# ArielElb/zkSnark-FinalProject

Measured on AMD Instinct MI355X. Metric: groth16_proofs_per_sec, higher is better.
Workload: dtype u32; 1 GPU; matrix-mul 128x128 + Poseidon MatrixCircuit: 10706932 constraints, 8675313 witness vars, domain 2^24; pk/R1CS/assignment resident in HBM; real key (zkg16_setup_resident) with window tables (zkg16_pk_precompute), last timed proof verified (zkg16_verify); parallelism=1 GPU

## Files before the change

zksnark-finalproject_amd/csrc/api.hip:

```cpp
#include <chrono>
#include <functional>
#include <thread>

#include <exception>

#include "common.hpp"
#include "group.hpp"

using namespace zk;

namespace zk {
ScopedKernelTimer::ScopedKernelTimer(zkg16_ctx *c, const char *n, double u, hipStream_t st)
    : ctx(c), name(n), units(u), stream(st ? st : c->stream) {
    if (!ctx->kernel_timing) return;
    if (ctx->kernel_timing_accumulate_only && strncmp(n, "msm_accumulate", 14) != 0) return;
    ZK_HIP(hipEventCreate(&e0));
    ZK_HIP(hipEventCreate(&e1));
    ZK_HIP(hipEventRecord(e0, stream));
}
ScopedKernelTimer::~ScopedKernelTimer() {
    if (!e0) return;
    (void)hipEventRecord(e1, stream);
    ctx->pending_events.push_back(PendingEvent{name, units, e0, e1});
}
// ... 31 lines not shown
    if (e.err == hipErrorInvalidValue && strstr(e.what, "domain")) return ZKG16_ERR_DOMAIN_TOO_LARGE;
    return ZKG16_ERR_HIP;
}

#define ZK_API_BEGIN(ctx)                         \
    if (!(ctx)) return ZKG16_ERR_BAD_ARG;         \
    std::lock_guard<std::mutex> _lk((ctx)->mu);   \
    try {                                         \
        ZK_HIP(hipSetDevice((ctx)->device));
#define ZK_API_END(ctx)                           \
    }                                             \
    catch (const HipError &e) { return fail((ctx), e); } \
    catch (const std::bad_alloc &) { return ZKG16_ERR_OOM; } \
    return ZKG16_OK;

void copy_options(zkg16_ctx *dst, const zkg16_ctx *src) {
    dst->opt_window_bits = src->opt_window_bits; dst->opt_min_seg = src->opt_min_seg; dst->opt_ntt_mode = src->opt_ntt_mode;
    dst->opt_reduce_mode = src->opt_reduce_mode; dst->opt_b_filter = src->opt_b_filter; dst->opt_spmv_dict = src->opt_spmv_dict;
    dst->opt_wm_first = src->opt_wm_first; dst->opt_g1_waves = src->opt_g1_waves; dst->opt_fixup_aux = src->opt_fixup_aux;
    dst->opt_window_bits_h = src->opt_window_bits_h; dst->opt_reduce_chunk = src->opt_reduce_chunk; dst->opt_wm_concurrent = src->opt_wm_concurrent;
    dst->opt_ntt_radix = src->opt_ntt_radix; dst->opt_ntt_xcd = src->opt_ntt_xcd; dst->opt_acc_debug = src->opt_acc_debug;
    dst->opt_sort_mode = src->opt_sort_mode; dst->opt_acc_pipeline = src->opt_acc_pipeline; dst->opt_fuse_pointwise = src->opt_fuse_pointwise;
    dst->opt_matrix_parts = src->opt_matrix_parts; dst->opt_g2_lazy = src->opt_g2_lazy; dst->opt_g1_inline = src->opt_g1_inline; dst->opt_fixed_base_bits = src->opt_fixed_base_bits;
    dst->opt_collect_threads = src->opt_collect_threads; dst->opt_batch_max = src->opt_batch_max; dst->opt_matrix_batch_threads = src->opt_matrix_batch_threads; dst->opt_matrix_batch_grid = src->opt_matrix_batch_grid; dst->opt_verify_batch_min = src->opt_verify_batch_min; dst->opt_verify_wire_min = src->opt_verify_wire_min; dst->opt_verify_each_after = src->opt_verify_each_after; dst->opt_wm_transforms = src->opt_wm_transforms;
    dst->kernel_timing = src->kernel_timing; dst->kernel_timing_accumulate_only = src->kernel_timing_accumulate_only;
}
void create_streams(zkg16_ctx *ctx) {
    ZK_HIP(hipStreamCreateWithFlags(&ctx->stream, hipStreamNonBlocking));
    ZK_HIP(hipStreamCreateWithFlags(&ctx->wm_stream, hipStreamNonBlocking));
    for (int i : {0, 2, 3, 4, 1}) ZK_HIP(hipStreamCreateWithFlags(&ctx->slots[i].stream, hipStreamNonBlocking));
}
void teardown(zkg16_ctx *ctx) {
    (void)hipStreamSynchronize(ctx->stream);
    (void)hipStreamSynchronize(ctx->wm_stream);
    if (ctx->extra_host) (void)hipHostFree(ctx->extra_host);
    if (ctx->batch_host) (void)hipHostFree(ctx->batch_host);
    ctx->batch_host = nullptr;
    ctx->batch_host_bytes = 0;
    if (ctx->mbatch_host) (void)hipHostFree(ctx->mbatch_host);
    ctx->mbatch_host = nullptr;
    ctx->mbatch_host_bytes = 0;
    ctx->mbatch_dev.release();
    if (ctx->circuit_stage) (void)hipHostFree(ctx->circuit_stage);
    ctx->circuit_stage = nullptr;
    ctx->circuit_stage_bytes = 0;
    for (int i = 0; i < 2; i++) {
        if (ctx->stage_host[i]) (void)hipHostFree(ctx->stage_host[i]);
// ... 939 lines not shown
        if (value < 0 || value > 15) return ZKG16_ERR_BAD_ARG;
        ctx->opt_acc_debug = (int)value;
        return ZKG16_OK;
    }
    if (!strcmp(name, "sort_mode")) {
        if (value < 0 || value > 1) return ZKG16_ERR_BAD_ARG;
        ctx->opt_sort_mode = (int)value;
        return ZKG16_OK;
    }
    if (!strcmp(name, "acc_pipeline")) {
        if (value < 0 || value > 4) return ZKG16_ERR_BAD_ARG;
        ctx->opt_acc_pipeline = value == 4 ? 0 : (int)value;
        return ZKG16_OK;
    }
    if (!strcmp(name, "fuse_pointwise")) {
        ctx->opt_fuse_pointwise = value ? 1 : 0;
        return ZKG16_OK;
    }
    if (!strcmp(name, "wm_transforms")) {
        if (value != 0 && value != 6 && value != 7) return ZKG16_ERR_BAD_ARG;
        ctx->opt_wm_transforms = value == 7 ? 7 : 6;
        return ZKG16_OK;
    }
    if (!strcmp(name, "wm_first")) {
        if (value < -1 || value > 2) return ZKG16_ERR_BAD_ARG;
        ctx->opt_wm_first = (int)value;
        return ZKG16_OK;
    }
    if (!strcmp(name, "spmv_dict")) {
        if (value < 0 || value > 2) return ZKG16_ERR_BAD_ARG;
        ctx->opt_spmv_dict = (int)value;
        return ZKG16_OK;
    }
    if (!strcmp(name, "b_filter")) {
        if (value < 0 || value > 2) return ZKG16_ERR_BAD_ARG;
        ctx->opt_b_filter = (int)value;
        return ZKG16_OK;
    }
    if (!strcmp(name, "collect_threads")) {
        if (value < 0 || value > 2) return ZKG16_ERR_BAD_ARG;
        ctx->opt_collect_threads = value == 0 ? -1 : value == 2 ? 0 : 1;
        return ZKG16_OK;
    }
    if (!strcmp(name, "fixed_base_bits")) {
        if (value != 0 && (value < 4 || value > 20 || (value > 14 && (value & 1)))) return ZKG16_ERR_BAD_ARG;
        ctx->opt_fixed_base_bits = (int)value;
// ... 1750 lines not shown
```

zksnark-finalproject_amd/csrc/common.hpp:

```cpp
#pragma once
#include <hip/hip_runtime.h>
#include <stdint.h>
#include <stdio.h>
#include <string.h>

#include <algorithm>
#include <array>
#include <atomic>
#include <condition_variable>
#include <functional>
#include <map>
#include <memory>
#include <mutex>
#include <shared_mutex>
#include <string>
#include <system_error>
#include <thread>
#include <vector>

#include "../../include/zkg16.h"
#include "ec.cuh"
#include "ff.cuh"

namespace zk {
// ... 58 lines not shown
    void ensure(size_t n) { if (n > bytes) alloc(n); }
    void release() { if (p) { dev_release(p, bytes); p = nullptr; bytes = 0; } }
    template <class T> T *as() const { return reinterpret_cast<T *>(p); }
};

struct FixedBaseCache {
    struct Entry { std::vector<uint8_t> key; DevBuf table; uint64_t stamp = 0; int wbits = 0; } e[2];
    uint64_t clock = 0;
    DevBuf sums, pref, win_bases, table_xyzz;
};

struct KernelStat { uint64_t launches = 0; double ms = 0, units = 0; };
struct PendingEvent;

struct NttTables {
    int log_n = 0;
    std::mutex mu;
    DevBuf w;
    DevBuf wu;
    DevBuf g;
    DevBuf gi;
    DevBuf g_u, gi_u;
    int u_passes = 0;
    Fr n_inv;
    Fr zinv;
};

struct PkDev {
    size_t num_instance = 0, m_total = 0;
    size_t z_lo = 0, z_hi = 0;
    size_t h_lo = 0, h_hi = 0, n_h_total = 0;
    DevBuf a, b1, l;
    DevBuf b2;
    DevBuf h;
    DevBuf b_mask;
    size_t b_skipped = 0;
    G1Affine alpha_g1, beta_g1, delta_g1;
    G2Affine beta_g2, delta_g2;
    bool blinding = true;
    bool full = true;
    int tab_c_z = 0, tab_c_h = 0;
};

struct R1csDev {
    size_t num_instance = 0, num_constraints = 0, num_variables = 0;
    int log_n = 0;
// ... 136 lines not shown
    int opt_ntt_mode = 1;
    int opt_reduce_mode = 3;
    int opt_b_filter = 0;
    int opt_spmv_dict = 0;
    int opt_wm_first = -1;
    int opt_g1_waves = 0;
    int opt_fixup_aux = 0;
    int opt_window_bits_h = 0;
    int opt_reduce_chunk = 0;
    int opt_wm_concurrent = -1;
    int opt_ntt_radix = 1;
    int opt_ntt_xcd = 1;
    int opt_acc_debug = 0;
    int opt_sort_mode = 0;
    int opt_acc_pipeline = 0;
    void *circuit_stage = nullptr;
    size_t circuit_stage_bytes = 0;
    int opt_collect_threads = -1;
    int opt_fixed_base_bits = 0;
    int opt_g2_lazy = 1;
    int opt_g1_inline = 1;
    int opt_matrix_parts = 0;
    int opt_fuse_pointwise = 1;
    int opt_wm_transforms = 6;
    int opt_batch_max = 0;
    int opt_matrix_batch_threads = 0;
    int opt_matrix_batch_grid = 0;
    int opt_verify_batch_min = ZKG16_VERIFY_BATCH_MIN_DEFAULT;
    int opt_verify_wire_min = ZKG16_VERIFY_WIRE_MIN_DEFAULT;
    int opt_verify_each_after = ZKG16_VERIFY_EACH_AFTER_DEFAULT;
    float vb_timings[11] = {0};
    int num_cus = 256;
    bool lds_attr_fixup[2] = {false, false}, lds_attr_ntt = false;
    zk::FixedBaseCache fb_g1, fb_g2;
    zk::DevBuf poseidon_dev;
    std::shared_ptr<zk::PrimeDev> prime_dev;
};

namespace zk {

struct PendingEvent { std::string name; double units; hipEvent_t e0, e1; };

struct ScopedKernelTimer {
    zkg16_ctx *ctx;
    const char *name;
    double units;
    hipEvent_t e0 = nullptr, e1 = nullptr;
    hipStream_t stream;
    ScopedKernelTimer(zkg16_ctx *c, const char *n, double u, hipStream_t st = nullptr);
    ~ScopedKernelTimer();
};
void kernel_timer_resolve(zkg16_ctx *ctx);

struct NttPointwise { const Fr *b, *c; Fr zinv; };
struct NttLast { const Fr *scale; bool pw_operand, sub; };
Fr *ntt_run(zkg16_ctx *ctx, Fr *src, Fr *dst, int log_n, bool inverse, bool coset, const NttPointwise *pw = nullptr,
            const NttLast *last = nullptr);
Fr *ntt_run_batch(zkg16_ctx *ctx, Fr *src, Fr *dst, int log_n, bool inverse, bool coset, const NttPointwise *pw, unsigned nvec, size_t vec_stride,
                  const NttLast *last = nullptr);
NttTables *ntt_get_tables(zkg16_ctx *ctx, int log_n);
struct NttShare {
    unsigned cols[4], rows[4];
    std::function<void()> between;
};
Fr *ntt_run_share(zkg16_ctx *ctx, Fr *src, Fr *dst, int log_n, bool inverse, bool coset, const NttPointwise *pw, const NttShare &share,
                  const NttLast *last = nullptr);
bool ntt_two_pass_shape(int log_n, int ntt_mode, int *log_n1, int *log_n2, int *tile_log);

struct SpmvRows { const uint32_t *list[3]; size_t n[3]; };
void spmv_run(zkg16_ctx *ctx, R1csDev &m, const Fr *z, Fr *a, Fr *b, Fr *c, const SpmvRows *rows = nullptr, const Fr *const *zs = nullptr,
              unsigned nvec = 1);
void pointwise_h_run(zkg16_ctx *ctx, Fr *ab_a, const Fr *b, const Fr *c , const Fr &zinv, size_t n);
void fr_from_mont_run(zkg16_ctx *ctx, const Fr *in, Fr *out, size_t n);
void witness_map_run(zkg16_ctx *ctx, R1csDev &m, const Fr *z, Fr **h_out);
void witness_map_run_batch(zkg16_ctx *ctx, R1csDev &m, const Fr *const *zs, unsigned nvec, Fr **h_out);

struct MsmPlan {
    size_t n = 0;
    int c = 0, nwin = 0;
    int nwin_digits = 0;
    bool tabled = false;
    size_t nb = 0;
    size_t total_entries = 0;
    uint32_t lanes_g1 = 0, lanes_g2 = 0;
    int batch = 1;
};
void msm_plan_build(zkg16_ctx *ctx, MsmWorkspace &ws, const Fr *scalars_canonical, size_t n, MsmPlan &plan, int window_bits = 0);
int msm_plan_bits(zkg16_ctx *ctx, size_t n, int window_bits, bool tabled);
size_t msm_plan_digits(zkg16_ctx *ctx, size_t n, int window_bits, bool tabled);
struct ScalarSrc { const Fr *main; size_t n_main; const Fr *extra; size_t n_extra; bool mont; const uint8_t *mask; const uint8_t *part = nullptr; int want_part = 0;
// ... 80 lines not shown
```

zksnark-finalproject_amd/csrc/ntt.hip:

```cpp
#include "common.hpp"
#include "fru.cuh"

namespace zk {

static constexpr int NTT_TILE_LOG = 11;
static constexpr int NTT_TILE = 1 << NTT_TILE_LOG;
static constexpr int NTT_THREADS = 256;
static constexpr int NTT_MAX_SUB_LOG = 11;

__device__ __forceinline__ int swz(int e) { return e ^ ((e >> 5) & 31); }

__device__ __forceinline__ Fr lds_ld(const uint32_t *s, int stride, int e) {
    Fr v;
    const int p = swz(e);
#pragma unroll
    for (int k = 0; k < 8; k++) v.l[k] = s[k * stride + p];
    return v;
}
__device__ __forceinline__ void lds_st(uint32_t *s, int stride, int e, const Fr &v) {
    const int p = swz(e);
#pragma unroll
    for (int k = 0; k < 8; k++) s[k * stride + p] = v.l[k];
}

// ... 20 lines not shown
__device__ __forceinline__ int bitrev(int x, int bits) { return bits == 0 ? 0 : (int)(__brev((unsigned)x) >> (32 - bits)); }

struct NttPassArgs {
    const Fr *in;
    Fr *out;
    const Fr *w;
    const uint32_t *wu;
    const Fr *pre;
    const Fr *pw_b, *pw_c;
    Fr pw_zinv;
    FrU pw_zc;
    const Fr *post;
    Fr post_const;
    int post_const_on;
    const Fr *sub;
    int log_n, log_n1, log_n2;
    int inverse;
    int tw_shift;
    size_t batch_stride;
    int out_stride_log;
    int xcd_order;
    unsigned tile_lo0, tile_n0, tile_lo1, tile_n1;
    size_t vec_stride;
};

__device__ __forceinline__ void vec_offset(NttPassArgs &a) {
    if (!blockIdx.z) return;
    const size_t vo = (size_t)blockIdx.z * a.vec_stride;
    a.in += vo;
    a.out += vo;
    if (a.pw_b) {
        a.pw_b += vo;
        if (a.pw_c) a.pw_c += vo;
    }
    if (a.sub) a.sub += vo;
}

__device__ __forceinline__ unsigned pass_tile(const NttPassArgs &a, unsigned group) {
    if (!a.tile_n0) return xcd_tile(blockIdx.x, gridDim.x, group);
    const unsigned t = xcd_tile(blockIdx.x, a.tile_n0 + a.tile_n1, group);
    return t < a.tile_n0 ? a.tile_lo0 + t : a.tile_lo1 + (t - a.tile_n0);
}

__device__ __forceinline__ void lds_dif(uint32_t *s_data, const uint32_t *s_tw, int log_m, int tw_stride) {
    const int tid = threadIdx.x;
    for (int s = log_m - 1; s >= 0; s--) {
        const int h = 1 << s;
        for (int u = tid; u < NTT_TILE / 2; u += NTT_THREADS) {
            const int c = u >> (log_m - 1);
            const int v = u & ((1 << (log_m - 1)) - 1);
            const int j = v & (h - 1);
            const int blk = v >> s;
            const int i0 = (c << log_m) + (blk << (s + 1)) + j;
            const int i1 = i0 + h;
            Fr a = lds_ld(s_data, NTT_TILE, i0);
            Fr b = lds_ld(s_data, NTT_TILE, i1);
            Fr sum = fp_add(a, b);
            Fr dif = fp_sub(a, b);
// ... 417 lines not shown
    if (!GTW) stage_twiddles_u(s_tw, tw_stride, a.w, a.log_n, a.log_n2, a.inverse);
    for (int t = threadIdx.x; t < TILE; t += NTT_THREADS_U) {
        const int i2 = t & ((1 << a.log_n2) - 1), r = t >> a.log_n2;
        FrU v;
#pragma unroll
        for (int k = 0; k < 9; k++) v.l[k] = 0;
        if (row0 + r < n1) v = load_u(a, in, (row0 + r) * n2 + i2);
        lds_st_u(s_data, TILE, t, v);
    }
    __syncthreads();
    lds_dif_u<TL, GTW, R4>(s_data, s_tw, a.log_n2, tw_stride, a);
    const FrU post_c = a.post_const_on ? fru_repack(a.post_const) : fru_one_sat();
    for (int t = threadIdx.x; t < TILE; t += NTT_THREADS_U) {
        const int r = t & (R - 1), k2 = t >> log_r;
        if (row0 + r >= n1) continue;
        const FrU v = lds_ld_u(s_data, TILE, (r << a.log_n2) + bitrev(k2, a.log_n2));
        const size_t k = (size_t)blockIdx.y + (((row0 + r) + n1 * (size_t)k2) << a.out_stride_log);
        Fr res = fru_mul_to_sat(v, a.post ? fru_repack(gld(a.post + k)) : post_c);
        if (a.sub) res = fp_sub(res, gld(a.sub + k));
        gst(a.out + k, res);
    }
}

__global__ void __launch_bounds__(256) ntt_wu_kernel(const Fr *w, uint32_t *wu, size_t n) {
    const size_t i = (size_t)blockIdx.x * blockDim.x + threadIdx.x;
    if (i >= n) return;
    const FrU u = fru_from_sat(gld(w + i));
#pragma unroll
    for (int k = 0; k < 9; k++) wu[i * 9 + k] = u.l[k];
}

static constexpr int FR_POWERS_RUN = 8;
__global__ void fr_powers_kernel(Fr *out, Fr base, Fr scale, size_t n) {
    const size_t i0 = ((size_t)blockIdx.x * blockDim.x + threadIdx.x) * FR_POWERS_RUN;
    if (i0 >= n) return;
    Fr cur = fp_mul(fp_pow_u64(base, (uint64_t)i0), scale);
    for (int k = 0; k < FR_POWERS_RUN && i0 + k < n; k++) {
        gst(out + i0 + k, cur);
        cur = fp_mul(cur, base);
    }
}
static unsigned fr_powers_grid(size_t n) { return (unsigned)(((n + FR_POWERS_RUN - 1) / FR_POWERS_RUN + 255) / 256); }

void fr_powers_run(zkg16_ctx *ctx, Fr *out, const Fr &base, const Fr &scale, size_t n) {
    if (!n) return;
    hipLaunchKernelGGL(fr_powers_kernel, dim3(fr_powers_grid(n)), dim3(256), 0, ctx->stream, out, base, scale, n);
// ... 28 lines not shown
    for (int i = 0; i < log_n; i++) gn = fp_sqr(gn);
    t->zinv = fp_inv(fp_sub(gn, Fr::one()));
    t->w.alloc(n * sizeof(Fr));
    t->g.alloc(n * sizeof(Fr));
    t->gi.alloc(n * sizeof(Fr));
    const int bs = 256;
    const unsigned grid = fr_powers_grid(n);
    hipLaunchKernelGGL(fr_powers_kernel, dim3(grid), dim3(bs), 0, ctx->stream, t->w.as<Fr>(), root, Fr::one(), n);
    hipLaunchKernelGGL(fr_powers_kernel, dim3(grid), dim3(bs), 0, ctx->stream, t->g.as<Fr>(), g, Fr::one(), n);
    hipLaunchKernelGGL(fr_powers_kernel, dim3(grid), dim3(bs), 0, ctx->stream, t->gi.as<Fr>(), g_inv, t->n_inv, n);
    ZK_HIP(hipGetLastError());
    ZK_HIP(hipStreamSynchronize(ctx->stream));
    NttTables *raw = t.get();
    owner->ntt_tables[log_n] = std::move(t);
    return raw;
}

static unsigned share_tiles(NttPassArgs &p, const unsigned t[4]) {
    if (!t[1]) throw HipError{hipErrorInvalidValue, "ntt: a share without tiles", __FILE__, __LINE__};
    p.tile_lo0 = t[0]; p.tile_n0 = t[1]; p.tile_lo1 = t[2]; p.tile_n1 = t[3];
    return t[1] + t[3];
}

static Fr *ntt_run_impl(zkg16_ctx *ctx, Fr *data, Fr *tmp, int log_n, bool inverse, bool coset, const NttPointwise *pw, const NttLast *last,
                        const NttShare *share, unsigned nvec = 1, size_t vec_stride = 0) {
    bool &lds_attr_set = ctx->lds_attr_ntt;
    if (!lds_attr_set) {
        for (const void *f : {reinterpret_cast<const void *>(ntt_pass_cols), reinterpret_cast<const void *>(ntt_pass_rows),
                              reinterpret_cast<const void *>(ntt_pass_cols_u<11, false, true>), reinterpret_cast<const void *>(ntt_pass_rows_u<11, false, true>),
                              reinterpret_cast<const void *>(ntt_pass_cols_u<12, true, true>), reinterpret_cast<const void *>(ntt_pass_rows_u<12, true, true>),
                              reinterpret_cast<const void *>(ntt_pass_cols_u<11, false, false>), reinterpret_cast<const void *>(ntt_pass_rows_u<11, false, false>),
                              reinterpret_cast<const void *>(ntt_pass_cols_u<12, true, false>), reinterpret_cast<const void *>(ntt_pass_rows_u<12, true, false>),
                              reinterpret_cast<const void *>(ntt_pass_cols_u<12, true, 2>), reinterpret_cast<const void *>(ntt_pass_rows_u<12, true, 2>),
                              reinterpret_cast<const void *>(ntt_pass_cols_u<11, false, 2>), reinterpret_cast<const void *>(ntt_pass_rows_u<11, false, 2>),
                              reinterpret_cast<const void *>(ntt_pass_cols_u<12, true, 3>), reinterpret_cast<const void *>(ntt_pass_rows_u<12, true, 3>),
                              reinterpret_cast<const void *>(ntt_pass_cols_u<11, false, 3>), reinterpret_cast<const void *>(ntt_pass_rows_u<11, false, 3>)})
            ZK_HIP(hipFuncSetAttribute(f, hipFuncAttributeMaxDynamicSharedMemorySize, 160 * 1024));
        lds_attr_set = true;
    }
    const bool uform = ctx->opt_ntt_mode != 0;
    const bool r4 = ctx->opt_ntt_radix == 4;
    const bool xch = ctx->opt_ntt_radix == 1;
    const bool xch2 = ctx->opt_ntt_radix == 3;
    auto *k_cols = uform ? (xch2 ? ntt_pass_cols_u<11, false, 3> : xch ? ntt_pass_cols_u<11, false, 2> : r4 ? ntt_pass_cols_u<11, false, true> : ntt_pass_cols_u<11, false, false>) : ntt_pass_cols;
    auto *k_rows = uform ? (xch2 ? ntt_pass_rows_u<11, false, 3> : xch ? ntt_pass_rows_u<11, false, 2> : r4 ? ntt_pass_rows_u<11, false, true> : ntt_pass_rows_u<11, false, false>) : ntt_pass_rows;
    const unsigned nthreads = uform ? NTT_THREADS_U : NTT_THREADS;
    if (log_n > 3 * NTT_MAX_SUB_LOG - 2) throw HipError{hipErrorInvalidValue, "ntt: domain above build limit 2^31", __FILE__, __LINE__};
    NttTables *t = ntt_get_tables(ctx, log_n);
    const size_t n = (size_t)1 << log_n;
    NttPassArgs a;
    memset(&a, 0, sizeof a);
    a.w = t->w.as<Fr>();
    a.log_n = log_n;
    a.inverse = inverse ? 1 : 0;
    a.xcd_order = ctx->opt_ntt_xcd;
    if (nvec < 1 || nvec > 65535 || (nvec > 1 && (share || vec_stride < n))) throw HipError{hipErrorInvalidValue, "ntt: bad batch of transforms", __FILE__, __LINE__};
    a.vec_stride = nvec > 1 ? vec_stride : 0;
    const Fr *pre = (!inverse && coset) ? t->g.as<Fr>() : nullptr;
    const Fr *post = (inverse && coset) ? t->gi.as<Fr>() : nullptr;
    int post_const_on = (inverse && !coset) ? 1 : 0;
    a.post_const = t->n_inv;
    if (uform) {
        const bool two_big = ctx->opt_ntt_mode != 3 && log_n > 2 * NTT_MAX_SUB_LOG && log_n <= 24;
        const int passes = log_n <= NTT_MAX_SUB_LOG ? 1 : (two_big || log_n <= 2 * NTT_MAX_SUB_LOG) ? 2 : 3;
        std::unique_lock<std::mutex> lazy(t->mu);
        if (t->u_passes != passes || !t->g_u.p) {
            DevBuf gu(n * sizeof(Fr)), giu(n * sizeof(Fr));
            const Fr g = fr_from_u64_host(7), g_inv = fp_inv(g);
            Fr back = fr_from_u64_host(1);
            for (int i = 0; i < 5 * passes; i++) back = fp_add(back, back);
            const unsigned grid = fr_powers_grid(n);
            hipLaunchKernelGGL(fr_powers_kernel, dim3(grid), dim3(256), 0, ctx->stream, gu.as<Fr>(), g, fr_from_u64_host(1024), n);
            hipLaunchKernelGGL(fr_powers_kernel, dim3(grid), dim3(256), 0, ctx->stream, giu.as<Fr>(), g_inv, fp_mul(t->n_inv, back), n);
            ZK_HIP(hipGetLastError());
            ZK_HIP(hipStreamSynchronize(ctx->stream));
            t->g_u = std::move(gu);
            t->gi_u = std::move(giu);
            t->u_passes = passes;
        }
        lazy.unlock();
        const int deficit = passes - (pre ? 1 : 0);
        Fr back = fr_from_u64_host(1);
        for (int i = 0; i < 5 * deficit; i++) back = fp_add(back, back);
        if (pre) pre = t->g_u.as<Fr>();
        if (post) post = t->gi_u.as<Fr>();
        a.post_const = post_const_on ? fp_mul(t->n_inv, back) : back;
        post_const_on = 1;
    }
    if (last && (last->scale || last->pw_operand)) {
        if (post) throw HipError{hipErrorInvalidValue, "ntt: a scaled last store of a coset ifft", __FILE__, __LINE__};
        Fr s = last->scale ? *last->scale : fr_from_u64_host(1);
        if (last->pw_operand && uform) s = fp_mul(s, fr_from_u64_host(32));
        a.post_const = post_const_on ? fp_mul(a.post_const, s) : s;
        post_const_on = 1;
    }
    Fr *const sub = (last && last->sub) ? tmp : nullptr;
    if (pw) {
        if (pre) throw HipError{hipErrorInvalidValue, "ntt: point-wise fusion needs a transform without a coset pre-multiply", __FILE__, __LINE__};
        a.pw_zinv = pw->zinv;
        a.pw_zc = fru_repack(fp_mul(pw->zinv, fr_from_u64_host((uint64_t)1 << 10)));
    }
    auto first = [&](NttPassArgs &p) {
        p.pre = pre;
        if (pw) { p.pw_b = pw->b; p.pw_c = pw->c; }
    };
    auto lds_bytes = [uform](int log_m) { return (size_t)(uform ? 9 : 8) * 4 * (NTT_TILE + (log_m > 0 ? (1 << (log_m - 1)) : 1)); };

    if (uform && ctx->opt_ntt_mode != 3 && log_n > 2 * NTT_MAX_SUB_LOG && log_n <= 24) {
        std::unique_lock<std::mutex> lazy(t->mu);
        if (!t->wu.p) {
            DevBuf wu(n * 9 * sizeof(uint32_t));
            hipLaunchKernelGGL(ntt_wu_kernel, dim3((unsigned)((n + 255) / 256)), dim3(256), 0, ctx->stream, t->w.as<Fr>(), wu.as<uint32_t>(), n);
            ZK_HIP(hipGetLastError());
            ZK_HIP(hipStreamSynchronize(ctx->stream));
            t->wu = std::move(wu);
        }
        lazy.unlock();
        a.wu = t->wu.as<uint32_t>();
        a.log_n2 = 12;
        a.log_n1 = log_n - 12;
        const size_t big_lds = (size_t)9 * 4 * 4096 + ((xch || xch2) ? 9 * 4 * 64 : 0);
        {
            NttPassArgs p1 = a;
            p1.in = data; p1.out = data;
            first(p1);
            p1.batch_stride = 0;
            const unsigned grid = share ? share_tiles(p1, share->cols) : (unsigned)(((size_t)1 << a.log_n2) >> (12 - a.log_n1));
            ScopedKernelTimer kt(ctx, "ntt_pass_cols", (double)n * nvec);
            const dim3 g(grid, 1, nvec);
            if (xch2) hipLaunchKernelGGL((ntt_pass_cols_u<12, true, 3>), g, dim3(NTT_THREADS_U), big_lds, ctx->stream, p1);
            else if (xch) hipLaunchKernelGGL((ntt_pass_cols_u<12, true, 2>), g, dim3(NTT_THREADS_U), big_lds, ctx->stream, p1);
            else if (r4) hipLaunchKernelGGL((ntt_pass_cols_u<12, true, true>), g, dim3(NTT_THREADS_U), big_lds, ctx->stream, p1);
            else hipLaunchKernelGGL((ntt_pass_cols_u<12, true, false>), g, dim3(NTT_THREADS_U), big_lds, ctx->stream, p1);
        }
        if (share) share->between();
        {
            NttPassArgs p2 = a;
            p2.in = data; p2.out = tmp;
            p2.post = post;
            p2.post_const_on = post_const_on;
            p2.sub = sub;
            const unsigned grid = share ? share_tiles(p2, share->rows) : (unsigned)((size_t)1 << a.log_n1);
            ScopedKernelTimer kt(ctx, "ntt_pass_rows", (double)n * nvec);
            const dim3 g(grid, 1, nvec);
            if (xch2) hipLaunchKernelGGL((ntt_pass_rows_u<12, true, 3>), g, dim3(NTT_THREADS_U), big_lds, ctx->stream, p2);
            else if (xch) hipLaunchKernelGGL((ntt_pass_rows_u<12, true, 2>), g, dim3(NTT_THREADS_U), big_lds, ctx->stream, p2);
            else if (r4) hipLaunchKernelGGL((ntt_pass_rows_u<12, true, true>), g, dim3(NTT_THREADS_U), big_lds, ctx->stream, p2);
            else hipLaunchKernelGGL((ntt_pass_rows_u<12, true, false>), g, dim3(NTT_THREADS_U), big_lds, ctx->stream, p2);
        }
    } else if (log_n <= NTT_MAX_SUB_LOG) {
        if (share) throw HipError{hipErrorInvalidValue, "ntt: a share of a single-pass transform", __FILE__, __LINE__};
        a.log_n1 = 0;
        a.log_n2 = log_n;
        a.in = data;
        a.out = tmp;
        first(a);
        a.post = post;
        a.post_const_on = post_const_on;
        a.sub = sub;
        ScopedKernelTimer kt(ctx, "ntt_pass_rows", (double)n * nvec);
        hipLaunchKernelGGL(k_rows, dim3(1, 1, nvec), dim3(nthreads), lds_bytes(log_n), ctx->stream, a);
    } else {
        const int log_m = log_n <= 2 * NTT_MAX_SUB_LOG ? log_n : 2 * NTT_MAX_SUB_LOG;
        const int log_n0 = log_n - log_m;
        if (share && log_n0 > 0) throw HipError{hipErrorInvalidValue, "ntt: a share of a three-pass transform", __FILE__, __LINE__};
        if (log_n0 > 0) {
            NttPassArgs p0 = a;
            p0.in = data; p0.out = data;
            first(p0);
            p0.log_n1 = log_n0; p0.log_n2 = log_m;
            const unsigned grid = (unsigned)(((size_t)1 << log_m) >> (NTT_TILE_LOG - log_n0));
            ScopedKernelTimer kt(ctx, "ntt_pass_cols", (double)n * nvec);
            hipLaunchKernelGGL(k_cols, dim3(grid, 1, nvec), dim3(nthreads), lds_bytes(log_n0), ctx->stream, p0);
        }
        a.log_n2 = log_m / 2;
        a.log_n1 = log_m - a.log_n2;
        const unsigned batches = 1u << log_n0;
        {
            NttPassArgs p1 = a;
            p1.in = data; p1.out = data;
            if (log_n0 == 0) first(p1);
            p1.tw_shift = log_n0;
            p1.batch_stride = (size_t)1 << log_m;
            const unsigned grid = share ? share_tiles(p1, share->cols) : (unsigned)(((size_t)1 << a.log_n2) >> (NTT_TILE_LOG - a.log_n1));
            ScopedKernelTimer kt(ctx, "ntt_pass_cols", (double)n * nvec);
            hipLaunchKernelGGL(k_cols, dim3(grid, batches, nvec), dim3(nthreads), lds_bytes(a.log_n1), ctx->stream, p1);
        }
        if (share) share->between();
        {
            NttPassArgs p2 = a;
            p2.in = data; p2.out = tmp;
            p2.post = post;
            p2.post_const_on = post_const_on;
            p2.sub = sub;
            p2.batch_stride = (size_t)1 << log_m;
            p2.out_stride_log = log_n0;
            const unsigned grid = share ? share_tiles(p2, share->rows) : (unsigned)(((size_t)1 << a.log_n1) >> (NTT_TILE_LOG - a.log_n2));
            ScopedKernelTimer kt(ctx, "ntt_pass_rows", (double)n * nvec);
            hipLaunchKernelGGL(k_rows, dim3(grid, batches, nvec), dim3(nthreads), lds_bytes(a.log_n2), ctx->stream, p2);
        }
    }
    ZK_HIP(hipGetLastError());
    return tmp;
}

Fr *ntt_run(zkg16_ctx *ctx, Fr *data, Fr *tmp, int log_n, bool inverse, bool coset, const NttPointwise *pw, const NttLast *last) {
    return ntt_run_impl(ctx, data, tmp, log_n, inverse, coset, pw, last, nullptr);
}
Fr *ntt_run_batch(zkg16_ctx *ctx, Fr *data, Fr *tmp, int log_n, bool inverse, bool coset, const NttPointwise *pw, unsigned nvec, size_t vec_stride,
                  const NttLast *last) {
    return ntt_run_impl(ctx, data, tmp, log_n, inverse, coset, pw, last, nullptr, nvec, vec_stride);
}

Fr *ntt_run_share(zkg16_ctx *ctx, Fr *data, Fr *tmp, int log_n, bool inverse, bool coset, const NttPointwise *pw, const NttShare &share,
                  const NttLast *last) {
    if (!ntt_two_pass_shape(log_n, ctx->opt_ntt_mode, nullptr, nullptr, nullptr))
        throw HipError{hipErrorInvalidValue, "ntt: a share of a transform that is not two-pass", __FILE__, __LINE__};
    return ntt_run_impl(ctx, data, tmp, log_n, inverse, coset, pw, last, &share);
}

bool ntt_two_pass_shape(int log_n, int ntt_mode, int *log_n1, int *log_n2, int *tile_log) {
    int l1, l2, tl;
    if (ntt_mode != 0 && ntt_mode != 3 && log_n > 2 * NTT_MAX_SUB_LOG && log_n <= 24) {
        l2 = 12; l1 = log_n - 12; tl = 12;
    } else if (log_n > NTT_MAX_SUB_LOG && log_n <= 2 * NTT_MAX_SUB_LOG) {
        l2 = log_n / 2; l1 = log_n - l2; tl = NTT_TILE_LOG;
    } else {
        return false;
    }
    if (log_n1) *log_n1 = l1;
    if (log_n2) *log_n2 = l2;
    if (tile_log) *tile_log = tl;
    return true;
}
// ... 3 lines not shown
```

zksnark-finalproject_amd/csrc/poly.hip:

```cpp
#include "common.hpp"

namespace zk {

__device__ __forceinline__ Fr gld_fr(const Fr *p) {
    const uint4 *q = reinterpret_cast<const uint4 *>(p);
    uint4 a = q[0], b = q[1];
    Fr v;
    v.l[0] = a.x; v.l[1] = a.y; v.l[2] = a.z; v.l[3] = a.w;
    v.l[4] = b.x; v.l[5] = b.y; v.l[6] = b.z; v.l[7] = b.w;
    return v;
}
__device__ __forceinline__ void gst_fr(Fr *p, const Fr &v) {
    uint4 *q = reinterpret_cast<uint4 *>(p);
    q[0] = make_uint4(v.l[0], v.l[1], v.l[2], v.l[3]);
    q[1] = make_uint4(v.l[4], v.l[5], v.l[6], v.l[7]);
}

struct SpmvArgs {
    const uint64_t *rp[3];
    const uint32_t *col[3];
    const uint32_t *perm[3];
    const Fr *cf[3];
    Fr *out[3];
    const Fr *z;
// ... 387 lines not shown
    ZK_HIP(hipGetLastError());
}

void pointwise_h_run(zkg16_ctx *ctx, Fr *ab_a, const Fr *b, const Fr *c, const Fr &zinv, size_t n) {
    ScopedKernelTimer kt(ctx, "pointwise_h_kernel", (double)n);
    hipLaunchKernelGGL(pointwise_h_kernel, dim3((unsigned)((n + 255) / 256)), dim3(256), 0, ctx->stream, ab_a, b, c, zinv, n);
    ZK_HIP(hipGetLastError());
}

void fr_from_mont_run(zkg16_ctx *ctx, const Fr *in, Fr *out, size_t n) {
    if (n == 0) return;
    ScopedKernelTimer kt(ctx, "fr_from_mont_kernel", (double)n);
    hipLaunchKernelGGL(fr_from_mont_kernel, dim3((unsigned)((n + 255) / 256)), dim3(256), 0, ctx->stream, in, out, n);
    ZK_HIP(hipGetLastError());
}

static Fr *wm_transforms(zkg16_ctx *ctx, int log_n, Fr *a, Fr *b, Fr *c, Fr *tmp, unsigned nvec) {
    const size_t n = (size_t)1 << log_n;
    auto run = [&](Fr *src, Fr *dst, bool inverse, bool coset, const NttPointwise *pw = nullptr, const NttLast *last = nullptr) {
        return ntt_run_batch(ctx, src, dst, log_n, inverse, coset, pw, nvec, n, last);
    };
    NttTables *t = ntt_get_tables(ctx, log_n);
    const bool fuse = ctx->opt_fuse_pointwise != 0;
    run(a, tmp, true, false);
    run(tmp, a, false, true);
    if (ctx->opt_wm_transforms == 7) {
        run(b, tmp, true, false);
        run(tmp, b, false, true);
        run(c, tmp, true, false);
        run(tmp, c, false, true);
        const NttPointwise pw{b, c, t->zinv};
        if (fuse) return run(a, tmp, true, true, &pw);
        pointwise_h_run(ctx, a, b, c, t->zinv, (size_t)nvec * n);
        return run(a, tmp, true, true);
    }
    const NttLast to_b{&t->zinv, fuse, false}, to_c{&t->zinv, false, false}, sub{nullptr, false, true};
    run(b, tmp, true, false);
    run(tmp, b, false, true, nullptr, &to_b);
    run(c, tmp, true, false, nullptr, &to_c);
    const NttPointwise pw{b, nullptr, t->zinv};
    if (fuse) return run(a, tmp, true, true, &pw, &sub);
    pointwise_h_run(ctx, a, b, nullptr, t->zinv, (size_t)nvec * n);
    return run(a, tmp, true, true, nullptr, &sub);
}

void witness_map_run(zkg16_ctx *ctx, R1csDev &m, const Fr *z, Fr **h_out) {
    const size_t n = (size_t)1 << m.log_n;
    for (int i = 0; i < 4; i++) ctx->poly[i].ensure(n * sizeof(Fr));
    Fr *a = ctx->poly[0].as<Fr>(), *b = ctx->poly[1].as<Fr>(), *c = ctx->poly[2].as<Fr>(), *tmp = ctx->poly[3].as<Fr>();
    spmv_run(ctx, m, z, a, b, c);
    *h_out = wm_transforms(ctx, m.log_n, a, b, c, tmp, 1);
}

void witness_map_run_batch(zkg16_ctx *ctx, R1csDev &m, const Fr *const *zs, unsigned nvec, Fr **h_out) {
    const size_t n = (size_t)1 << m.log_n;
    for (int i = 0; i < 4; i++) ctx->poly[i].ensure((size_t)nvec * n * sizeof(Fr));
    Fr *a = ctx->poly[0].as<Fr>(), *b = ctx->poly[1].as<Fr>(), *c = ctx->poly[2].as<Fr>(), *tmp = ctx->poly[3].as<Fr>();
    spmv_run(ctx, m, nullptr, a, b, c, nullptr, zs, nvec);
    *h_out = wm_transforms(ctx, m.log_n, a, b, c, tmp, nvec);
}
// ... 3 lines not shown
```

Baseline: 6.860 proofs/s.

## Fuse adjacent NTT row/column passes across witness-map transforms

Adds a fused kernel that runs an inverse NTT's row pass and the following coset forward NTT's column pass in one launch. The coset multiply and twiddle fold into a per-element operand (either a precomputed power table or the pointwise operand). The six-transform witness map is rescheduled into column, join and row parts with swapped split shapes, and this path is on by default. A second mode instead folds the coset pre-multiply into the previous inverse's post-scale. The goal is to remove full-domain global memory round trips between passes, at the cost of new lazily built tables and more complex index and layout bookkeeping.

```diff
diff --git a/zksnark-finalproject_amd/csrc/api.hip b/zksnark-finalproject_amd/csrc/api.hip
--- a/zksnark-finalproject_amd/csrc/api.hip
+++ b/zksnark-finalproject_amd/csrc/api.hip
@@ -77,7 +77,7 @@
     dst->opt_ntt_radix = src->opt_ntt_radix; dst->opt_ntt_xcd = src->opt_ntt_xcd; dst->opt_acc_debug = src->opt_acc_debug;
     dst->opt_sort_mode = src->opt_sort_mode; dst->opt_acc_pipeline = src->opt_acc_pipeline; dst->opt_fuse_pointwise = src->opt_fuse_pointwise;
     dst->opt_matrix_parts = src->opt_matrix_parts; dst->opt_g2_lazy = src->opt_g2_lazy; dst->opt_g1_inline = src->opt_g1_inline; dst->opt_fixed_base_bits = src->opt_fixed_base_bits;
-    dst->opt_collect_threads = src->opt_collect_threads; dst->opt_batch_max = src->opt_batch_max; dst->opt_matrix_batch_threads = src->opt_matrix_batch_threads; dst->opt_matrix_batch_grid = src->opt_matrix_batch_grid; dst->opt_verify_batch_min = src->opt_verify_batch_min; dst->opt_verify_wire_min = src->opt_verify_wire_min; dst->opt_verify_each_after = src->opt_verify_each_after; dst->opt_wm_transforms = src->opt_wm_transforms;
+    dst->opt_collect_threads = src->opt_collect_threads; dst->opt_batch_max = src->opt_batch_max; dst->opt_matrix_batch_threads = src->opt_matrix_batch_threads; dst->opt_matrix_batch_grid = src->opt_matrix_batch_grid; dst->opt_verify_batch_min = src->opt_verify_batch_min; dst->opt_verify_wire_min = src->opt_verify_wire_min; dst->opt_verify_each_after = src->opt_verify_each_after; dst->opt_wm_transforms = src->opt_wm_transforms; dst->opt_wm_fuse = src->opt_wm_fuse;
     dst->kernel_timing = src->kernel_timing; dst->kernel_timing_accumulate_only = src->kernel_timing_accumulate_only;
 }
 void create_streams(zkg16_ctx *ctx) {
@@ -1063,6 +1063,11 @@
         ctx->opt_wm_transforms = value == 7 ? 7 : 6;
         return ZKG16_OK;
     }
+    if (!strcmp(name, "wm_fuse")) {
+        if (value < -1 || value > 2) return ZKG16_ERR_BAD_ARG;
+        ctx->opt_wm_fuse = value < 0 ? 1 : (int)value;
+        return ZKG16_OK;
+    }
     if (!strcmp(name, "wm_first")) {
         if (value < -1 || value > 2) return ZKG16_ERR_BAD_ARG;
         ctx->opt_wm_first = (int)value;
diff --git a/zksnark-finalproject_amd/csrc/common.hpp b/zksnark-finalproject_amd/csrc/common.hpp
--- a/zksnark-finalproject_amd/csrc/common.hpp
+++ b/zksnark-finalproject_amd/csrc/common.hpp
@@ -104,6 +104,8 @@
     DevBuf gi;
     DevBuf g_u, gi_u;
     int u_passes = 0;
+    DevBuf gf_u;
+    DevBuf gn_u;
     Fr n_inv;
     Fr zinv;
 };
@@ -286,6 +288,7 @@
     int opt_g1_inline = 1;
     int opt_matrix_parts = 0;
     int opt_fuse_pointwise = 1;
+    int opt_wm_fuse = 1;
     int opt_wm_transforms = 6;
     int opt_batch_max = 0;
     int opt_matrix_batch_threads = 0;
@@ -317,7 +320,7 @@
 void kernel_timer_resolve(zkg16_ctx *ctx);
 
 struct NttPointwise { const Fr *b, *c; Fr zinv; };
-struct NttLast { const Fr *scale; bool pw_operand, sub; };
+struct NttLast { const Fr *scale; bool pw_operand, sub, coset_next, coset_done; };
 Fr *ntt_run(zkg16_ctx *ctx, Fr *src, Fr *dst, int log_n, bool inverse, bool coset, const NttPointwise *pw = nullptr,
             const NttLast *last = nullptr);
 Fr *ntt_run_batch(zkg16_ctx *ctx, Fr *src, Fr *dst, int log_n, bool inverse, bool coset, const NttPointwise *pw, unsigned nvec, size_t vec_stride,
@@ -330,6 +333,14 @@
 Fr *ntt_run_share(zkg16_ctx *ctx, Fr *src, Fr *dst, int log_n, bool inverse, bool coset, const NttPointwise *pw, const NttShare &share,
                   const NttLast *last = nullptr);
 bool ntt_two_pass_shape(int log_n, int ntt_mode, int *log_n1, int *log_n2, int *tile_log);
+struct NttPart {
+    enum What { COLS, ROWS, JOIN } what;
+    bool swapped;
+    const Fr *operand;
+};
+Fr *ntt_run_part(zkg16_ctx *ctx, Fr *src, Fr *dst, int log_n, bool inverse, bool coset, const NttPart &part, unsigned nvec, size_t vec_stride,
+                 const NttLast *last = nullptr);
+bool ntt_parts_available(zkg16_ctx *ctx, int log_n);
 
 struct SpmvRows { const uint32_t *list[3]; size_t n[3]; };
 void spmv_run(zkg16_ctx *ctx, R1csDev &m, const Fr *z, Fr *a, Fr *b, Fr *c, const SpmvRows *rows = nullptr, const Fr *const *zs = nullptr,
diff --git a/zksnark-finalproject_amd/csrc/ntt.hip b/zksnark-finalproject_amd/csrc/ntt.hip
--- a/zksnark-finalproject_amd/csrc/ntt.hip
+++ b/zksnark-finalproject_amd/csrc/ntt.hip
@@ -66,6 +66,8 @@
     int xcd_order;
     unsigned tile_lo0, tile_n0, tile_lo1, tile_n1;
     size_t vec_stride;
+    const Fr *mid;
+    int mid_per_vec, inverse2;
 };
 
 __device__ __forceinline__ void vec_offset(NttPassArgs &a) {
@@ -78,6 +80,7 @@
         if (a.pw_c) a.pw_c += vo;
     }
     if (a.sub) a.sub += vo;
+    if (a.mid && a.mid_per_vec) a.mid += vo;
 }
 
 __device__ __forceinline__ unsigned pass_tile(const NttPassArgs &a, unsigned group) {
@@ -541,6 +544,55 @@
     }
 }
 
+template <int TL, bool GTW, int R4>
+__global__ void __launch_bounds__(NTT_THREADS_U) ntt_pass_rows_cols_u(NttPassArgs a) {
+    constexpr int TILE = 1 << TL;
+    constexpr int PER = TILE / NTT_THREADS_U;
+    extern __shared__ __attribute__((aligned(16))) uint32_t smem[];
+    uint32_t *s_data = smem;
+    uint32_t *s_tw = smem + 9 * TILE;
+    const int tw_stride = 1 << (a.log_n2 - 1);
+    const int log_r = TL - a.log_n2;
+    const int R = 1 << log_r;
+    const unsigned nmask = (1u << a.log_n) - 1u;
+    const size_t n1 = (size_t)1 << a.log_n1;
+    const size_t n2 = (size_t)1 << a.log_n2;
+    const size_t row0 = (size_t)pass_tile(a, (R >= 4 || !a.xcd_order) ? 1u : 4u / (unsigned)R) * R;
+    vec_offset(a);
+
+    if (!GTW) stage_twiddles_u(s_tw, tw_stride, a.w, a.log_n, a.log_n2, a.inverse);
+    for (int t = threadIdx.x; t < TILE; t += NTT_THREADS_U) lds_st_u(s_data, TILE, t, load_u(a, a.in, row0 * n2 + t));
+    __syncthreads();
+    lds_dif_u<TL, GTW, R4>(s_data, s_tw, a.log_n2, tw_stride, a);
+    FrU v[PER];
+#pragma unroll
+    for (int q = 0; q < PER; q++) {
+        const int t = threadIdx.x + q * NTT_THREADS_U;
+        const int r = t & (R - 1), k2 = t >> log_r;
+        const FrU x = lds_ld_u(s_data, TILE, (r << a.log_n2) + bitrev(k2, a.log_n2));
+        v[q] = fru_mul(x, fru_repack(gld(a.mid + ((row0 + r) + n1 * (size_t)k2))));
+    }
+    __syncthreads();
+#pragma unroll
+    for (int q = 0; q < PER; q++) {
+        const int t = threadIdx.x + q * NTT_THREADS_U;
+        const int r = t & (R - 1), k2 = t >> log_r;
+        lds_st_u(s_data, TILE, (r << a.log_n2) + k2, v[q]);
+    }
+    a.inverse = a.inverse2;
+    if (!GTW) stage_twiddles_u(s_tw, tw_stride, a.w, a.log_n, a.log_n2, a.inverse);
+    __syncthreads();
+    lds_dif_u<TL, GTW, R4>(s_data, s_tw, a.log_n2, tw_stride, a);
+    for (int t = threadIdx.x; t < TILE; t += NTT_THREADS_U) {
+        const int c = t & (R - 1), k1 = t >> log_r;
+        const FrU x = lds_ld_u(s_data, TILE, (c << a.log_n2) + bitrev(k1, a.log_n2));
+        const size_t i2 = row0 + c;
+        unsigned e = (unsigned)((i2 * (size_t)k1) & nmask);
+        if (a.inverse) e = ((1u << a.log_n) - e) & nmask;
+        gst(a.out + (size_t)k1 * n1 + i2, fru_mul_to_sat(x, fru_repack(gld(a.w + e))));
+    }
+}
+
 __global__ void __launch_bounds__(256) ntt_wu_kernel(const Fr *w, uint32_t *wu, size_t n) {
     const size_t i = (size_t)blockIdx.x * blockDim.x + threadIdx.x;
     if (i >= n) return;
@@ -615,8 +667,14 @@
     return t[1] + t[3];
 }
 
+using NttPassKernel = void (*)(NttPassArgs);
+static NttPassKernel ntt_fused_kernel(bool big, int radix) {
+    if (big) return radix == 3 ? ntt_pass_rows_cols_u<12, true, 3> : radix == 1 ? ntt_pass_rows_cols_u<12, true, 2> : radix == 4 ? ntt_pass_rows_cols_u<12, true, 1> : ntt_pass_rows_cols_u<12, true, 0>;
+    return radix == 3 ? ntt_pass_rows_cols_u<11, false, 3> : radix == 1 ? ntt_pass_rows_cols_u<11, false, 2> : radix == 4 ? ntt_pass_rows_cols_u<11, false, 1> : ntt_pass_rows_cols_u<11, false, 0>;
+}
+
 static Fr *ntt_run_impl(zkg16_ctx *ctx, Fr *data, Fr *tmp, int log_n, bool inverse, bool coset, const NttPointwise *pw, const NttLast *last,
-                        const NttShare *share, unsigned nvec = 1, size_t vec_stride = 0) {
+                        const NttShare *share, unsigned nvec = 1, size_t vec_stride = 0, const NttPart *part = nullptr) {
     bool &lds_attr_set = ctx->lds_attr_ntt;
     if (!lds_attr_set) {
         for (const void *f : {reinterpret_cast<const void *>(ntt_pass_cols), reinterpret_cast<const void *>(ntt_pass_rows),
@@ -629,6 +687,9 @@
                               reinterpret_cast<const void *>(ntt_pass_cols_u<12, true, 3>), reinterpret_cast<const void *>(ntt_pass_rows_u<12, true, 3>),
                               reinterpret_cast<const void *>(ntt_pass_cols_u<11, false, 3>), reinterpret_cast<const void *>(ntt_pass_rows_u<11, false, 3>)})
             ZK_HIP(hipFuncSetAttribute(f, hipFuncAttributeMaxDynamicSharedMemorySize, 160 * 1024));
+        for (int big = 0; big < 2; big++)
+            for (int radix = 1; radix <= 4; radix++)
+                ZK_HIP(hipFuncSetAttribute(reinterpret_cast<const void *>(ntt_fused_kernel(big != 0, radix)), hipFuncAttributeMaxDynamicSharedMemorySize, 160 * 1024));
         lds_attr_set = true;
     }
     const bool uform = ctx->opt_ntt_mode != 0;
@@ -639,6 +700,10 @@
     auto *k_rows = uform ? (xch2 ? ntt_pass_rows_u<11, false, 3> : xch ? ntt_pass_rows_u<11, false, 2> : r4 ? ntt_pass_rows_u<11, false, true> : ntt_pass_rows_u<11, false, false>) : ntt_pass_rows;
     const unsigned nthreads = uform ? NTT_THREADS_U : NTT_THREADS;
     if (log_n > 3 * NTT_MAX_SUB_LOG - 2) throw HipError{hipErrorInvalidValue, "ntt: domain above build limit 2^31", __FILE__, __LINE__};
+    if (part && (!uform || share || !ntt_two_pass_shape(log_n, ctx->opt_ntt_mode, nullptr, nullptr, nullptr) ||
+                 (part->what == NttPart::JOIN && (pw || last || (part->operand ? (inverse || !coset) : (!inverse || coset))))))
+        throw HipError{hipErrorInvalidValue, "ntt: a part of a transform that has no such part", __FILE__, __LINE__};
+    const bool do_cols = !part || part->what == NttPart::COLS, do_rows = !part || part->what == NttPart::ROWS;
     NttTables *t = ntt_get_tables(ctx, log_n);
     const size_t n = (size_t)1 << log_n;
     NttPassArgs a;
@@ -649,7 +714,11 @@
     a.xcd_order = ctx->opt_ntt_xcd;
     if (nvec < 1 || nvec > 65535 || (nvec > 1 && (share || vec_stride < n))) throw HipError{hipErrorInvalidValue, "ntt: bad batch of transforms", __FILE__, __LINE__};
     a.vec_stride = nvec > 1 ? vec_stride : 0;
-    const Fr *pre = (!inverse && coset) ? t->g.as<Fr>() : nullptr;
+    const bool coset_next = last && last->coset_next, coset_done = last && last->coset_done;
+    if ((coset_next || coset_done) && (!uform || share || !ntt_two_pass_shape(log_n, ctx->opt_ntt_mode, nullptr, nullptr, nullptr) ||
+                                       (coset_next ? (!inverse || coset || last->scale) : (inverse || !coset))))
+        throw HipError{hipErrorInvalidValue, "ntt: no folded coset pre-multiply for this transform", __FILE__, __LINE__};
+    const Fr *pre = (!inverse && coset && !coset_done) ? t->g.as<Fr>() : nullptr;
     const Fr *post = (inverse && coset) ? t->gi.as<Fr>() : nullptr;
     int post_const_on = (inverse && !coset) ? 1 : 0;
     a.post_const = t->n_inv;
@@ -671,12 +740,31 @@
             t->gi_u = std::move(giu);
             t->u_passes = passes;
         }
+        if (coset_next && !t->gf_u.p) {
+            DevBuf gfu(n * sizeof(Fr));
+            Fr sc = t->n_inv;
+            for (int i = 0; i < 5 * passes; i++) sc = fp_add(sc, sc);
+            hipLaunchKernelGGL(fr_powers_kernel, dim3(fr_powers_grid(n)), dim3(256), 0, ctx->stream, gfu.as<Fr>(), fr_from_u64_host(7), sc, n);
+            ZK_HIP(hipGetLastError());
+            ZK_HIP(hipStreamSynchronize(ctx->stream));
+            t->gf_u = std::move(gfu);
+        }
+        if (part && part->what == NttPart::JOIN && !part->operand && !t->gn_u.p) {
+            DevBuf gnu(n * sizeof(Fr));
+            Fr sc = t->n_inv;
+            for (int i = 0; i < 5 * passes + 5; i++) sc = fp_add(sc, sc);
+            hipLaunchKernelGGL(fr_powers_kernel, dim3(fr_powers_grid(n)), dim3(256), 0, ctx->stream, gnu.as<Fr>(), fr_from_u64_host(7), sc, n);
+            ZK_HIP(hipGetLastError());
+            ZK_HIP(hipStreamSynchronize(ctx->stream));
+            t->gn_u = std::move(gnu);
+        }
         lazy.unlock();
         const int deficit = passes - (pre ? 1 : 0);
         Fr back = fr_from_u64_host(1);
         for (int i = 0; i < 5 * deficit; i++) back = fp_add(back, back);
         if (pre) pre = t->g_u.as<Fr>();
         if (post) post = t->gi_u.as<Fr>();
+        if (coset_next) post = t->gf_u.as<Fr>();
         a.post_const = post_const_on ? fp_mul(t->n_inv, back) : back;
         post_const_on = 1;
     }
@@ -698,6 +786,16 @@
         if (pw) { p.pw_b = pw->b; p.pw_c = pw->c; }
     };
     auto lds_bytes = [uform](int log_m) { return (size_t)(uform ? 9 : 8) * 4 * (NTT_TILE + (log_m > 0 ? (1 << (log_m - 1)) : 1)); };
+    auto join = [&](int tile_log, size_t lds) {
+        NttPassArgs pj = a;
+        pj.in = data; pj.out = tmp;
+        pj.mid = part->operand ? part->operand : t->gn_u.as<Fr>();
+        pj.mid_per_vec = part->operand ? 1 : 0;
+        pj.inverse2 = inverse ? 0 : 1;
+        const unsigned grid = (unsigned)(((size_t)1 << a.log_n1) >> (tile_log - a.log_n2));
+        ScopedKernelTimer kt(ctx, "ntt_pass_rows_cols", (double)n * nvec);
+        hipLaunchKernelGGL(ntt_fused_kernel(tile_log == 12, ctx->opt_ntt_radix), dim3(grid, 1, nvec), dim3(NTT_THREADS_U), lds, ctx->stream, pj);
+    };
 
     if (uform && ctx->opt_ntt_mode != 3 && log_n > 2 * NTT_MAX_SUB_LOG && log_n <= 24) {
         std::unique_lock<std::mutex> lazy(t->mu);
@@ -712,8 +810,9 @@
         a.wu = t->wu.as<uint32_t>();
         a.log_n2 = 12;
         a.log_n1 = log_n - 12;
+        if (part && part->swapped) std::swap(a.log_n1, a.log_n2);
         const size_t big_lds = (size_t)9 * 4 * 4096 + ((xch || xch2) ? 9 * 4 * 64 : 0);
-        {
+        if (do_cols) {
             NttPassArgs p1 = a;
             p1.in = data; p1.out = data;
             first(p1);
@@ -727,13 +826,13 @@
             else hipLaunchKernelGGL((ntt_pass_cols_u<12, true, false>), g, dim3(NTT_THREADS_U), big_lds, ctx->stream, p1);
         }
         if (share) share->between();
-        {
+        if (do_rows) {
             NttPassArgs p2 = a;
             p2.in = data; p2.out = tmp;
             p2.post = post;
             p2.post_const_on = post_const_on;
             p2.sub = sub;
-            const unsigned grid = share ? share_tiles(p2, share->rows) : (unsigned)((size_t)1 << a.log_n1);
+            const unsigned grid = share ? share_tiles(p2, share->rows) : (unsigned)(((size_t)1 << a.log_n1) >> (12 - a.log_n2));
             ScopedKernelTimer kt(ctx, "ntt_pass_rows", (double)n * nvec);
             const dim3 g(grid, 1, nvec);
             if (xch2) hipLaunchKernelGGL((ntt_pass_rows_u<12, true, 3>), g, dim3(NTT_THREADS_U), big_lds, ctx->stream, p2);
@@ -741,6 +840,7 @@
             else if (r4) hipLaunchKernelGGL((ntt_pass_rows_u<12, true, true>), g, dim3(NTT_THREADS_U), big_lds, ctx->stream, p2);
             else hipLaunchKernelGGL((ntt_pass_rows_u<12, true, false>), g, dim3(NTT_THREADS_U), big_lds, ctx->stream, p2);
         }
+        if (part && part->what == NttPart::JOIN) join(12, big_lds);
     } else if (log_n <= NTT_MAX_SUB_LOG) {
         if (share) throw HipError{hipErrorInvalidValue, "ntt: a share of a single-pass transform", __FILE__, __LINE__};
         a.log_n1 = 0;
@@ -768,8 +868,9 @@
         }
         a.log_n2 = log_m / 2;
         a.log_n1 = log_m - a.log_n2;
+        if (part && part->swapped) std::swap(a.log_n1, a.log_n2);
         const unsigned batches = 1u << log_n0;
-        {
+        if (do_cols) {
             NttPassArgs p1 = a;
             p1.in = data; p1.out = data;
             if (log_n0 == 0) first(p1);
@@ -780,7 +881,7 @@
             hipLaunchKernelGGL(k_cols, dim3(grid, batches, nvec), dim3(nthreads), lds_bytes(a.log_n1), ctx->stream, p1);
         }
         if (share) share->between();
-        {
+        if (do_rows) {
             NttPassArgs p2 = a;
             p2.in = data; p2.out = tmp;
             p2.post = post;
@@ -792,9 +893,10 @@
             ScopedKernelTimer kt(ctx, "ntt_pass_rows", (double)n * nvec);
             hipLaunchKernelGGL(k_rows, dim3(grid, batches, nvec), dim3(nthreads), lds_bytes(a.log_n2), ctx->stream, p2);
         }
+        if (part && part->what == NttPart::JOIN) join(NTT_TILE_LOG, lds_bytes(a.log_n2));
     }
     ZK_HIP(hipGetLastError());
-    return tmp;
+    return (part && part->what == NttPart::COLS) ? data : tmp;
 }
 
 Fr *ntt_run(zkg16_ctx *ctx, Fr *data, Fr *tmp, int log_n, bool inverse, bool coset, const NttPointwise *pw, const NttLast *last) {
@@ -803,6 +905,14 @@
 Fr *ntt_run_batch(zkg16_ctx *ctx, Fr *data, Fr *tmp, int log_n, bool inverse, bool coset, const NttPointwise *pw, unsigned nvec, size_t vec_stride,
                   const NttLast *last) {
     return ntt_run_impl(ctx, data, tmp, log_n, inverse, coset, pw, last, nullptr, nvec, vec_stride);
+}
+
+Fr *ntt_run_part(zkg16_ctx *ctx, Fr *data, Fr *tmp, int log_n, bool inverse, bool coset, const NttPart &part, unsigned nvec, size_t vec_stride,
+                 const NttLast *last) {
+    return ntt_run_impl(ctx, data, tmp, log_n, inverse, coset, nullptr, last, nullptr, nvec, vec_stride, &part);
+}
+bool ntt_parts_available(zkg16_ctx *ctx, int log_n) {
+    return ctx->opt_ntt_mode != 0 && ntt_two_pass_shape(log_n, ctx->opt_ntt_mode, nullptr, nullptr, nullptr);
 }
 
 Fr *ntt_run_share(zkg16_ctx *ctx, Fr *data, Fr *tmp, int log_n, bool inverse, bool coset, const NttPointwise *pw, const NttShare &share,
diff --git a/zksnark-finalproject_amd/csrc/poly.hip b/zksnark-finalproject_amd/csrc/poly.hip
--- a/zksnark-finalproject_amd/csrc/poly.hip
+++ b/zksnark-finalproject_amd/csrc/poly.hip
@@ -433,9 +433,15 @@
     };
     NttTables *t = ntt_get_tables(ctx, log_n);
     const bool fuse = ctx->opt_fuse_pointwise != 0;
-    run(a, tmp, true, false);
-    run(tmp, a, false, true);
-    if (ctx->opt_wm_transforms == 7) {
+    const bool six = ctx->opt_wm_transforms != 7;
+    const bool parts = six && ctx->opt_wm_fuse == 1 && fuse && ntt_parts_available(ctx, log_n);
+    const bool fold = six && ctx->opt_wm_fuse == 2 && ntt_parts_available(ctx, log_n);
+    const NttLast fold_next{nullptr, false, false, true, false}, fold_done{nullptr, false, false, false, true};
+    if (!parts) {
+        run(a, tmp, true, false, nullptr, fold ? &fold_next : nullptr);
+        run(tmp, a, false, true, nullptr, fold ? &fold_done : nullptr);
+    }
+    if (!six) {
         run(b, tmp, true, false);
         run(tmp, b, false, true);
         run(c, tmp, true, false);
@@ -445,8 +451,23 @@
         pointwise_h_run(ctx, a, b, c, t->zinv, (size_t)nvec * n);
         return run(a, tmp, true, true);
     }
-    const NttLast to_b{&t->zinv, fuse, false}, to_c{&t->zinv, false, false}, sub{nullptr, false, true};
-    run(b, tmp, true, false);
+    const NttLast to_b{&t->zinv, fuse, false, false, fold}, to_c{&t->zinv, false, false}, sub{nullptr, false, true};
+    if (parts) {
+        auto part = [&](Fr *src, Fr *dst, bool inverse, bool coset, NttPart::What what, bool swapped, const Fr *operand = nullptr,
+                        const NttLast *last = nullptr) {
+            return ntt_run_part(ctx, src, dst, log_n, inverse, coset, NttPart{what, swapped, operand}, nvec, n, last);
+        };
+        part(a, a, true, false, NttPart::COLS, false);
+        part(a, tmp, true, false, NttPart::JOIN, false);
+        part(b, b, true, false, NttPart::COLS, false);
+        part(b, a, true, false, NttPart::JOIN, false);
+        part(a, b, false, true, NttPart::ROWS, true, nullptr, &to_b);
+        part(tmp, a, false, true, NttPart::JOIN, true, b);
+        part(c, c, true, false, NttPart::COLS, false);
+        part(c, tmp, true, false, NttPart::ROWS, false, nullptr, &to_c);
+        return part(a, tmp, true, true, NttPart::ROWS, false, nullptr, &sub);
+    }
+    run(b, tmp, true, false, nullptr, fold ? &fold_next : nullptr);
     run(tmp, b, false, true, nullptr, &to_b);
     run(c, tmp, true, false, nullptr, &to_c);
     const NttPointwise pw{b, nullptr, t->zinv};
```

Result: no change. 6.923 proofs/s (median of 6 runs) (+0.9%).
